# zeyadmohamedabdo/Visual-Question-Answering-VQA-system

Hardware: AMD Instinct MI355X
Metric: image-question pairs/sec (train step) (higher is better)
Workload: dtype bf16; 1 GPU; VQA train step fwd+CE+bwd+allreduce+clip+AdamW, batch 512/GPU, 3x224x224 images, 20 tokens, d=256, 4 text layers, 49 image tokens, 1000 answers, dropout on (BASELINE configs[2]); batch_per_gpu=512, global_batch=512, parallelism=dp1, reducer=off

## Files before the change

visual-question-answering-vqa-system_amd/csrc/token_ops.hip:

```cpp
#include <cstdlib>
#include "common.h"

template <typename T>
__global__ void embed_fwd_kernel(const long long* __restrict__ ids, const float* __restrict__ emb, const float* __restrict__ pe,
                                 T* __restrict__ out, int rows, int L, int D, int V, float scale, float p, uint64_t seed) {
  seed = drop_resolve(seed);
  const size_t i = (size_t)blockIdx.x * blockDim.x + threadIdx.x;
  if (i >= (size_t)rows * D) return;
  const int d = (int)(i % D), row = (int)(i / D), l = row % L;
  long long id = ids[row];
  float v = (id >= 0 && id < V) ? emb[(size_t)id * D + d] * scale : 0.f;
  v += pe[(size_t)l * D + d];
  if (p > 0.f) v = drop_keep32(drop_key(seed), (uint32_t)(i), p) ? v / (1.f - p) : 0.f;
  out[i] = from_f<T>(v);
}
__global__ __launch_bounds__(1024) void fold_rows_kernel(const float* __restrict__ part, int nrows, size_t stride, int ncols,
                                                         float* dst0, int n0, float* dst1) {
  const int c = blockIdx.x * 64 + threadIdx.x, rg = threadIdx.y;
  const int per = (nrows + 15) / 16, r0 = rg * per, r1 = min(nrows, r0 + per);
  float t = 0.f;
  if (c < ncols) {
    int r = r0;
    for (; r + 16 <= r1; r += 16) {
      float v[16];
// ... 802 lines not shown
  DT(hipLaunchKernelGGL((attn_fwd_kernel<float, true>), dim3(B * H), dim3(256), shm, st, (const float*)q, (const float*)k, (const float*)v, ldq, ldk, ldv, kmask, probs, (float*)ctx, ldc, H, Lq, Lk, hd, scale, 0.f, 0ull, kv_index, n_kv),
     hipLaunchKernelGGL((attn_fwd_kernel<bf16_t, true>), dim3(B * H), dim3(256), shm, st, (const bf16_t*)q, (const bf16_t*)k, (const bf16_t*)v, ldq, ldk, ldv, kmask, probs, (bf16_t*)ctx, ldc, H, Lq, Lk, hd, scale, 0.f, 0ull, kv_index, n_kv));
  VQA_LAUNCH_CHECK(); return VQA_OK;
}
int vqa_attention_bwd(int dtype, const void* dctx, int ldc, const void* q, const void* k, const void* v, int ldq, int ldk, int ldv,
                      const float* probs, void* dq, void* dk, void* dv, int lddq, int lddk, int lddv,
                      int B, int H, int Lq, int Lk, int hd, float p, unsigned long long seed, hipStream_t st) {
  return attention_bwd_valu<false>(dtype, dctx, ldc, q, k, v, ldq, ldk, ldv, probs, nullptr, dq, dk, dv, lddq, lddk, lddv, B, H, Lq, Lk, hd, p, seed, st);
}
int vqa_attention_bwd_dp(int dtype, const void* dctx, int ldc, const void* q, const void* k, const void* v, int ldq, int ldk, int ldv,
                         const float* probs, const float* dprobs, void* dq, void* dk, void* dv, int lddq, int lddk, int lddv,
                         int B, int H, int Lq, int Lk, int hd, float p, unsigned long long seed, hipStream_t st) {
  if (!dprobs) return VQA_EARG;
  return attention_bwd_valu<true>(dtype, dctx, ldc, q, k, v, ldq, ldk, ldv, probs, dprobs, dq, dk, dv, lddq, lddk, lddv, B, H, Lq, Lk, hd, p, seed, st);
}
int vqa_masked_pool_fwd(int dtype, const void* x, const float* mask, void* out, int ldo, int col0, int B, int L, int D, hipStream_t st) {
  DT(hipLaunchKernelGGL(masked_pool_fwd_kernel<float>, dim3(B), dim3(256), 0, st, (const float*)x, mask, (float*)out, ldo, col0, L, D),
     hipLaunchKernelGGL(masked_pool_fwd_kernel<bf16_t>, dim3(B), dim3(256), 0, st, (const bf16_t*)x, mask, (bf16_t*)out, ldo, col0, L, D));
  VQA_LAUNCH_CHECK(); return VQA_OK;
}
int vqa_masked_pool_pair_fwd(int dtype, const void* x0, const void* x1, const float* mask, void* out, int B, int L, int D, hipStream_t st) {
  if (!x0 || !x1 || !out || B <= 0 || L <= 0 || D <= 0) return VQA_EARG;
  DT(hipLaunchKernelGGL(masked_pool_pair_fwd_kernel<float>, dim3(B, 2), dim3(256), 0, st, (const float*)x0, (const float*)x1, mask, (float*)out, L, D),
     hipLaunchKernelGGL(masked_pool_pair_fwd_kernel<bf16_t>, dim3(B, 2), dim3(256), 0, st, (const bf16_t*)x0, (const bf16_t*)x1, mask, (bf16_t*)out, L, D));
  VQA_LAUNCH_CHECK(); return VQA_OK;
}
int vqa_masked_pool_pair_bwd(int dtype, const void* dcat, const float* mask, void* dx0, void* dx1, int B, int L, int D, hipStream_t st) {
  if (!dcat || !dx0 || !dx1 || B <= 0 || L <= 0 || D <= 0) return VQA_EARG;
  DT(hipLaunchKernelGGL(masked_pool_pair_bwd_kernel<float>, dim3(B, 2), dim3(256), 0, st, (const float*)dcat, mask, (float*)dx0, (float*)dx1, L, D),
     hipLaunchKernelGGL(masked_pool_pair_bwd_kernel<bf16_t>, dim3(B, 2), dim3(256), 0, st, (const bf16_t*)dcat, mask, (bf16_t*)dx0, (bf16_t*)dx1, L, D));
  VQA_LAUNCH_CHECK(); return VQA_OK;
}
int vqa_masked_pool_bwd(int dtype, const void* dpool, int ldo, int col0, const float* mask, const void* addend, void* dx, int B, int L, int D, hipStream_t st) {
  DT(hipLaunchKernelGGL(masked_pool_bwd_kernel<float>, dim3(B), dim3(256), 0, st, (const float*)dpool, ldo, col0, mask, (const float*)addend, (float*)dx, L, D),
     hipLaunchKernelGGL(masked_pool_bwd_kernel<bf16_t>, dim3(B), dim3(256), 0, st, (const bf16_t*)dpool, ldo, col0, mask, (const bf16_t*)addend, (bf16_t*)dx, L, D));
  VQA_LAUNCH_CHECK(); return VQA_OK;
}
int vqa_gate_fwd(int dtype, const void* z, const void* cat, void* fused, int B, int D, hipStream_t st) {
  DT(hipLaunchKernelGGL(gate_fwd_kernel<float>, dim3(g1((size_t)B * D)), dim3(256), 0, st, (const float*)z, (const float*)cat, (float*)fused, B, D),
     hipLaunchKernelGGL(gate_fwd_kernel<bf16_t>, dim3(g1((size_t)B * D)), dim3(256), 0, st, (const bf16_t*)z, (const bf16_t*)cat, (bf16_t*)fused, B, D));
  VQA_LAUNCH_CHECK(); return VQA_OK;
}
int vqa_gate_bwd(int dtype, const void* dfused, const void* z, const void* cat, void* dz, void* dcat, int B, int D, hipStream_t st) {
  DT(hipLaunchKernelGGL(gate_bwd_kernel<float>, dim3(g1((size_t)B * D)), dim3(256), 0, st, (const float*)dfused, (const float*)z, (const float*)cat, (float*)dz, (float*)dcat, B, D),
     hipLaunchKernelGGL(gate_bwd_kernel<bf16_t>, dim3(g1((size_t)B * D)), dim3(256), 0, st, (const bf16_t*)dfused, (const bf16_t*)z, (const bf16_t*)cat, (bf16_t*)dz, (bf16_t*)dcat, B, D));
  VQA_LAUNCH_CHECK(); return VQA_OK;
}
int vqa_grad_tap_add(int dtype, const float* g, void* acc, int rows, int cols, int ld, int layout, hipStream_t st) {
  if (!g || !acc || rows < 0 || cols <= 0 || ld <= 0) return VQA_EARG;
  if (rows == 0) return VQA_OK;
  if (layout == 0) {
    if (ld < cols) return VQA_EARG;
    const size_t n = (size_t)rows * cols;
    DT(hipLaunchKernelGGL(grad_tap_rows_kernel<float>, dim3(g1(n)), dim3(256), 0, st, g, (float*)acc, cols, ld, n),
       hipLaunchKernelGGL(grad_tap_rows_kernel<bf16_t>, dim3(g1(n)), dim3(256), 0, st, g, (bf16_t*)acc, cols, ld, n));
  } else if (layout == 1) {
    if (rows % ld) return VQA_EARG;
    const int B = rows / ld;
    if (B > 65535) return VQA_EARG;
    const dim3 grid((unsigned)((ld + 31) / 32), (unsigned)((cols + 63) / 64), (unsigned)B);
    DT(hipLaunchKernelGGL(grad_tap_nchw_kernel<float>, grid, dim3(256), 0, st, g, (float*)acc, cols, ld),
       hipLaunchKernelGGL(grad_tap_nchw_kernel<bf16_t>, grid, dim3(256), 0, st, g, (bf16_t*)acc, cols, ld));
  } else {
    return VQA_EARG;
  }
  VQA_LAUNCH_CHECK(); return VQA_OK;
}
int vqa_add(int dtype, const void* a, const void* b, void* out, long long n, hipStream_t st) {
  DT(hipLaunchKernelGGL(add_kernel<float>, dim3(g1((size_t)n)), dim3(256), 0, st, (const float*)a, (const float*)b, (float*)out, (size_t)n),
     hipLaunchKernelGGL(add_kernel<bf16_t>, dim3(g1((size_t)n)), dim3(256), 0, st, (const bf16_t*)a, (const bf16_t*)b, (bf16_t*)out, (size_t)n));
  VQA_LAUNCH_CHECK(); return VQA_OK;
}
struct BiasBwdGeom { bool vec; int gpb, rows_per; dim3 grid; };
static BiasBwdGeom bias_bwd_geom(int dtype, int M, int N) {
  BiasBwdGeom g;
  const int VEC = dtype ? 8 : 4;
  g.vec = N % VEC == 0 && M > 0 && (256 % (N / VEC < 256 ? N / VEC : 256)) == 0;
  if (g.vec) {
    const int cvs = N / VEC, gpb = cvs < 256 ? cvs : 256, lanes_r = 256 / gpb;
    int gy = (M + 4 * lanes_r - 1) / (4 * lanes_r);
    if (gy > 1024) gy = 1024;
    if (gy < 1) gy = 1;
    g.gpb = gpb; g.rows_per = (M + gy - 1) / gy;
    g.grid = dim3((cvs + gpb - 1) / gpb, (M + g.rows_per - 1) / g.rows_per);
  } else {
    int gy = (M + 127) / 128; if (gy > 256) gy = 256; if (gy < 1) gy = 1;
    g.gpb = 0; g.rows_per = 0; g.grid = dim3((N + 63) / 64, gy);
  }
  return g;
}
long long vqa_bias_act_bwd_ws(int dtype, int M, int N) {
  if (M <= 0 || N <= 0) return 0;
  const BiasBwdGeom g = bias_bwd_geom(dtype, M, N);
  return (long long)g.grid.y * N;
}
int vqa_bias_act_bwd_fold_rows(int dtype, int M, int N) {
  if (M <= 0 || N <= 0) return 0;
  return (int)bias_bwd_geom(dtype, M, N).grid.y;
}
int vqa_bias_act_bwd(int dtype, const void* dout, const void* outact, void* dz, float* dbias, int M, int N, float p, unsigned long long seed,
                     float* ws, int defer_fold, hipStream_t st) {
  if (M <= 0 || N <= 0 || (defer_fold && !ws)) return VQA_EARG;
  const BiasBwdGeom g = bias_bwd_geom(dtype, M, N);
  if (g.vec) {
    DT(hipLaunchKernelGGL(bias_act_bwd_vec_kernel<float>, g.grid, dim3(256), 0, st, (const float*)dout, (const float*)outact, (float*)dz, dbias, M, N, p, seed, g.rows_per, ws),
       hipLaunchKernelGGL(bias_act_bwd_vec_kernel<bf16_t>, g.grid, dim3(256), 0, st, (const bf16_t*)dout, (const bf16_t*)outact, (bf16_t*)dz, dbias, M, N, p, seed, g.rows_per, ws));
  } else {
    DT(hipLaunchKernelGGL(bias_act_bwd_kernel<float>, g.grid, dim3(256), 0, st, (const float*)dout, (const float*)outact, (float*)dz, dbias, M, N, 0, p, seed, ws),
       hipLaunchKernelGGL(bias_act_bwd_kernel<bf16_t>, g.grid, dim3(256), 0, st, (const bf16_t*)dout, (const bf16_t*)outact, (bf16_t*)dz, dbias, M, N, 0, p, seed, ws));
  }
  if (ws && dbias && !defer_fold) launch_fold(ws, (int)g.grid.y, (size_t)N, N, dbias, N, nullptr, st);
  VQA_LAUNCH_CHECK(); return VQA_OK;
}
int vqa_fold_group(int njobs, const float* const* part, const int* nrows, const long long* stride, const int* ncols, float* const* dst0,
                   const int* n0, float* const* dst1, hipStream_t st) {
  if (njobs <= 0 || !part || !nrows || !stride || !ncols || !dst0 || !n0 || !dst1) return VQA_EARG;
  for (int base = 0; base < njobs; base += FOLD_MAXJOBS) {
    FoldGroup g;
    g.n = njobs - base < FOLD_MAXJOBS ? njobs - base : FOLD_MAXJOBS;
    g.blk0[0] = 0;
    for (int q = 0; q < g.n; ++q) {
      const int j = base + q;
      if (!part[j] || !dst0[j] || nrows[j] <= 0 || ncols[j] <= 0 || stride[j] <= 0 || stride[j] > 0xffffffffll || (n0[j] < ncols[j] && !dst1[j]))
        return VQA_EARG;
      g.j[q] = FoldJob{part[j], dst0[j], dst1[j], nrows[j], ncols[j], n0[j], (unsigned)stride[j]};
      g.blk0[q + 1] = g.blk0[q] + (ncols[j] + 63) / 64;
    }
    hipLaunchKernelGGL(fold_group_kernel, dim3(g.blk0[g.n]), dim3(64, 16), 0, st, g);
  }
  VQA_LAUNCH_CHECK(); return VQA_OK;
}
int vqa_cross_entropy(int dtype, const void* logits, const long long* targets, float* loss, void* dlogits, float* logits_f32, int B, int N,
                      float gscale, int* err, float* ws, hipStream_t st) {
  if (!logits || !targets || B <= 0 || N <= 0) return VQA_EARG;
  dim3 grid((B + 3) / 4);
  DT(hipLaunchKernelGGL(cross_entropy_kernel<float>, grid, dim3(256), 0, st, (const float*)logits, targets, loss, (float*)dlogits, logits_f32, B, N, gscale, err, ws),
     hipLaunchKernelGGL(cross_entropy_kernel<bf16_t>, grid, dim3(256), 0, st, (const bf16_t*)logits, targets, loss, (bf16_t*)dlogits, logits_f32, B, N, gscale, err, ws));
  if (ws && loss) launch_fold(ws, B, 1, 1, loss, 1, nullptr, st);
  VQA_LAUNCH_CHECK(); return VQA_OK;
}
int vqa_convert(int dtype_in, int dtype_out, const void* in, void* out, long long n, hipStream_t st) {
  const unsigned g = g1((size_t)n);
  if (!dtype_in && dtype_out) hipLaunchKernelGGL((convert_kernel<float, bf16_t>), dim3(g), dim3(256), 0, st, (const float*)in, (bf16_t*)out, (size_t)n);
  else if (dtype_in && !dtype_out) hipLaunchKernelGGL((convert_kernel<bf16_t, float>), dim3(g), dim3(256), 0, st, (const bf16_t*)in, (float*)out, (size_t)n);
  else if (!dtype_in) hipLaunchKernelGGL((convert_kernel<float, float>), dim3(g), dim3(256), 0, st, (const float*)in, (float*)out, (size_t)n);
  else hipLaunchKernelGGL((convert_kernel<bf16_t, bf16_t>), dim3(g), dim3(256), 0, st, (const bf16_t*)in, (bf16_t*)out, (size_t)n);
  VQA_LAUNCH_CHECK(); return VQA_OK;
}

}

typedef __attribute__((ext_vector_type(16))) float f32x16;

template <int HD, int NKT, int WPB, bool IDX = false>
__global__ __launch_bounds__(WPB * 64, 1) void attn_fwd_mfma_kernel(const bf16_t* __restrict__ q, const bf16_t* __restrict__ k, const bf16_t* __restrict__ v,
                                                            int ldq, int ldk, int ldv, const float* __restrict__ kmask, float* __restrict__ probs,
                                                            bf16_t* __restrict__ ctx, int ldc, int BH, int H, int Lq, int Lk, float p, uint64_t seed,
                                                            const int* __restrict__ kv_index, int n_kv) {
  seed = drop_resolve(seed);
  constexpr int LDV = HD;
  constexpr int KR = NKT * 32;
  constexpr int LDP = KR + 1;
  extern __shared__ __attribute__((aligned(16))) char smem[];
  const int lane = threadIdx.x & 63, wave = threadIdx.x >> 6;
  const int bh = blockIdx.x * WPB + wave;
  bf16_t* Vs = reinterpret_cast<bf16_t*>(smem) + wave * (KR * LDV);
  float* Ps = reinterpret_cast<float*>(smem + WPB * KR * LDV * 2) + wave * (32 * LDP);
  if (bh >= BH) return;
  const int b = bh / H, h = bh - b * H;
  const int r = lane & 31, hh = lane >> 5;
  const float inv_scale = 1.0f / sqrtf((float)HD);
  int kb = b;
  if constexpr (IDX) {
    kb = __builtin_amdgcn_readfirstlane(kv_index[b]);
    if (kb < 0 || kb >= n_kv) {
      for (int i = lane; i < Lq * Lk; i += 64) probs[(size_t)bh * Lq * Lk + i] = NAN;
      for (int i = lane; i < Lq * HD; i += 64) ctx[(size_t)(b * Lq + i / HD) * ldc + h * HD + i % HD] = f2bf(NAN);
      return;
    }
  }

  for (int i = lane; i < KR * (HD / 8); i += 64) {
    const int row = i / (HD / 8), cv = i - row * (HD / 8);
    u32x4 val = {0u, 0u, 0u, 0u};
    if (row < Lk) val = *reinterpret_cast<const u32x4*>(v + (size_t)(kb * Lk + row) * ldv + h * HD + cv * 8);
    *reinterpret_cast<u32x4*>(&Vs[row * LDV + cv * 8]) = val;
  }
  f32x16 st[NKT];
#pragma unroll
  for (int t = 0; t < NKT; ++t)
#pragma unroll
    for (int e = 0; e < 16; ++e) st[t][e] = 0.f;
#pragma unroll
  for (int ks = 0; ks < HD / 16; ++ks) {
    bf16x8 qf = {};
    if (r < Lq) qf = *reinterpret_cast<const bf16x8*>(q + (size_t)(b * Lq + r) * ldq + h * HD + ks * 16 + 8 * hh);
#pragma unroll
    for (int t = 0; t < NKT; ++t) {
      bf16x8 kf = {};
      if (32 * t + r < Lk) kf = *reinterpret_cast<const bf16x8*>(k + (size_t)(kb * Lk + 32 * t + r) * ldk + h * HD + ks * 16 + 8 * hh);
      st[t] = __builtin_amdgcn_mfma_f32_32x32x16_bf16(kf, qf, st[t], 0, 0, 0);
    }
  }
  float m = -INFINITY;
#pragma unroll
  for (int t = 0; t < NKT; ++t)
#pragma unroll
    for (int e = 0; e < 16; ++e) {
      const int key = 32 * t + (e & 3) + 8 * (e >> 2) + 4 * hh;
      float s = st[t][e] * inv_scale;
      if (key >= Lk || (kmask && kmask[kb * Lk + key] == 0.f)) s = -INFINITY;
      st[t][e] = s;
      m = fmaxf(m, s);
    }
  m = fmaxf(m, __shfl_xor(m, 32, 64));
  float sum = 0.f;
#pragma unroll
  for (int t = 0; t < NKT; ++t)
#pragma unroll
    for (int e = 0; e < 16; ++e) { const float ex = expf(st[t][e] - m); st[t][e] = ex; sum += ex; }
  sum += __shfl_xor(sum, 32, 64);
  const float rs = 1.0f / sum;
  const size_t prow = ((size_t)bh * Lq + r) * Lk;
#pragma unroll
  for (int t = 0; t < NKT; ++t)
#pragma unroll
    for (int e = 0; e < 16; ++e) {
      const int key = 32 * t + (e & 3) + 8 * (e >> 2) + 4 * hh;
      float pr = st[t][e] * rs;
      if (sum != sum || m != m) pr = st[t][e] / sum;
      Ps[r * LDP + key] = pr;
      if (p > 0.f && r < Lq && key < Lk) pr = drop_keep32(drop_key(seed), (uint32_t)(prow + key), p) ? pr / (1.f - p) : 0.f;
      st[t][e] = pr;
    }
  asm volatile("s_waitcnt lgkmcnt(0)" ::: "memory");
  for (int i = lane; i < Lq * Lk; i += 64) { const int qi = i / Lk, kj = i - qi * Lk; probs[(size_t)bh * Lq * Lk + i] = Ps[qi * LDP + kj]; }
  f32x16 o[HD / 32];
#pragma unroll
  for (int c = 0; c < HD / 32; ++c)
#pragma unroll
    for (int e = 0; e < 16; ++e) o[c][e] = 0.f;
  const int g2 = (lane >> 4) & 1, li = lane & 15, qd = li >> 2, pp = li & 3;
  typedef __attribute__((ext_vector_type(8))) short i16x8;
#pragma unroll
  for (int t = 0; t < NKT; ++t)
#pragma unroll
    for (int s = 0; s < 2; ++s) {
      bf16x8 af;
#pragma unroll
      for (int jj = 0; jj < 8; ++jj) af[jj] = (__bf16)st[t][8 * s + jj];
#pragma unroll
      for (int c = 0; c < HD / 32; ++c) {
        const bf16_t* vb = Vs + (32 * t + 16 * s + 4 * hh + qd) * LDV + c * 32 + 16 * g2 + 4 * pp;
        i16x4 lo = __builtin_amdgcn_ds_read_tr16_b64_v4i16((i16x4 __attribute__((address_space(3)))*)(vb));
        i16x4 hi = __builtin_amdgcn_ds_read_tr16_b64_v4i16((i16x4 __attribute__((address_space(3)))*)(vb + 8 * LDV));
        i16x8 tt = {lo[0], lo[1], lo[2], lo[3], hi[0], hi[1], hi[2], hi[3]};
        o[c] = __builtin_amdgcn_mfma_f32_32x32x16_bf16(af, __builtin_bit_cast(bf16x8, tt), o[c], 0, 0, 0);
      }
    }
#pragma unroll
  for (int c = 0; c < HD / 32; ++c)
#pragma unroll
    for (int e = 0; e < 16; ++e) {
      const int qi = (e & 3) + 8 * (e >> 2) + 4 * hh;
      if (qi < Lq) ctx[(size_t)(b * Lq + qi) * ldc + h * HD + c * 32 + r] = f2bf(o[c][e]);
    }
}

extern "C" int vqa_attention_fwd_mfma(const void* q, const void* k, const void* v, int ldq, int ldk, int ldv, const float* kmask, float* probs,
                                      void* ctx, int ldc, int B, int H, int Lq, int Lk, int hd, float p, unsigned long long seed, hipStream_t st) {
  if (!q || !k || !v || !probs || !ctx || Lq > 32 || Lk > 160 || (hd != 32 && hd != 64) || (ldq % 8) || (ldk % 8) || (ldv % 8)) return VQA_EARG;
  const int BH = B * H;
  auto go = [&](auto kern, int nkt, int wpb) {
    const size_t shm = (size_t)wpb * (nkt * 32) * hd * 2 + (size_t)wpb * 32 * (nkt * 32 + 1) * 4;
    (void)vqa_ensure_lds(reinterpret_cast<const void*>(kern), shm);
    hipLaunchKernelGGL(kern, dim3((BH + wpb - 1) / wpb), dim3(wpb * 64), shm, st, (const bf16_t*)q, (const bf16_t*)k, (const bf16_t*)v, ldq, ldk, ldv,
                       kmask, probs, (bf16_t*)ctx, ldc, BH, H, Lq, Lk, p, seed, nullptr, 0);
  };
  if (Lk <= 64) { if (hd == 32) go(&attn_fwd_mfma_kernel<32, 2, 4>, 2, 4); else go(&attn_fwd_mfma_kernel<64, 2, 4>, 2, 4); }
  else { if (hd == 32) go(&attn_fwd_mfma_kernel<32, 5, 2>, 5, 2); else go(&attn_fwd_mfma_kernel<64, 5, 2>, 5, 2); }
  VQA_LAUNCH_CHECK(); return VQA_OK;
}

extern "C" int vqa_attention_fwd_mfma_idx(const void* q, const void* k, const void* v, int ldq, int ldk, int ldv, const int* kv_index, int n_kv,
                                          const float* kmask, float* probs, void* ctx, int ldc, int B, int H, int Lq, int Lk, int hd, hipStream_t st) {
  if (!q || !k || !v || !kv_index || n_kv < 0 || !probs || !ctx || Lq > 32 || Lk > 160 || (hd != 32 && hd != 64) || (ldq % 8) || (ldk % 8) || (ldv % 8))
    return VQA_EARG;
  const int BH = B * H;
  auto go = [&](auto kern, int nkt, int wpb) {
    const size_t shm = (size_t)wpb * (nkt * 32) * hd * 2 + (size_t)wpb * 32 * (nkt * 32 + 1) * 4;
    (void)vqa_ensure_lds(reinterpret_cast<const void*>(kern), shm);
    hipLaunchKernelGGL(kern, dim3((BH + wpb - 1) / wpb), dim3(wpb * 64), shm, st, (const bf16_t*)q, (const bf16_t*)k, (const bf16_t*)v, ldq, ldk, ldv,
                       kmask, probs, (bf16_t*)ctx, ldc, BH, H, Lq, Lk, 0.f, 0ull, kv_index, n_kv);
  };
  if (Lk <= 64) { if (hd == 32) go(&attn_fwd_mfma_kernel<32, 2, 4, true>, 2, 4); else go(&attn_fwd_mfma_kernel<64, 2, 4, true>, 2, 4); }
  else { if (hd == 32) go(&attn_fwd_mfma_kernel<32, 5, 2, true>, 5, 2); else go(&attn_fwd_mfma_kernel<64, 5, 2, true>, 5, 2); }
  VQA_LAUNCH_CHECK(); return VQA_OK;
}

template <int HD>
__device__ __forceinline__ bf16x8 attn_ldsB(const bf16_t* tile, int row0, int c, int hh, int g2, int qd, int pp) {
  typedef __attribute__((ext_vector_type(8))) short i16x8;
  const bf16_t* vb = tile + (row0 + 4 * hh + qd) * HD + c * 32 + 16 * g2 + 4 * pp;
  i16x4 lo = __builtin_amdgcn_ds_read_tr16_b64_v4i16((i16x4 __attribute__((address_space(3)))*)(vb));
  i16x4 hi = __builtin_amdgcn_ds_read_tr16_b64_v4i16((i16x4 __attribute__((address_space(3)))*)(vb + 8 * HD));
  i16x8 tt = {lo[0], lo[1], lo[2], lo[3], hi[0], hi[1], hi[2], hi[3]};
  return __builtin_bit_cast(bf16x8, tt);
}

template <int HD, int NKT, int WPB, bool DPR>
__global__ __launch_bounds__(WPB * 64, 1) void attn_bwd_mfma_kernel(const bf16_t* __restrict__ dctx, int ldc, const bf16_t* __restrict__ q,
                                                            const bf16_t* __restrict__ k, const bf16_t* __restrict__ v, int ldq, int ldk, int ldv,
                                                            const float* __restrict__ probs, bf16_t* __restrict__ dq, bf16_t* __restrict__ dk,
                                                            bf16_t* __restrict__ dv, int lddq, int lddk, int lddv, int BH, int H, int Lq, int Lk,
                                                            float p, uint64_t seed, const float* __restrict__ dprobs) {
  seed = drop_resolve(seed);
  constexpr int KR = NKT * 32;
  constexpr int LDP = KR + 1;
  constexpr int WAVE_BYTES = (KR + 32 + 32) * HD * 2 + 32 * LDP * 4 + 32 * 4 + (DPR ? 32 * LDP * 4 : 0);
  extern __shared__ __attribute__((aligned(16))) char smem[];
  const int lane = threadIdx.x & 63, wave = threadIdx.x >> 6;
  const int bh = blockIdx.x * WPB + wave;
  if (bh >= BH) return;
  char* base = smem + (size_t)wave * WAVE_BYTES;
  bf16_t* Ks = reinterpret_cast<bf16_t*>(base);
  bf16_t* Qs = Ks + KR * HD;
  bf16_t* Os = Qs + 32 * HD;
  float* Ps = reinterpret_cast<float*>(Os + 32 * HD);
  float* Ts = Ps + 32 * LDP;
  float* DPs = Ts + 32;
  const int b = bh / H, h = bh - b * H;
  const int r = lane & 31, hh = lane >> 5;
  const int g2 = (lane >> 4) & 1, li = lane & 15, qd = li >> 2, pp = li & 3;
  const float inv_scale = 1.0f / sqrtf((float)HD);
  const float keep = p > 0.f ? 1.f / (1.f - p) : 1.f;

  for (int i = lane; i < KR * (HD / 8); i += 64) {
    const int row = i / (HD / 8), cv = i - row * (HD / 8);
    u32x4 val = {0u, 0u, 0u, 0u};
    if (row < Lk) val = *reinterpret_cast<const u32x4*>(k + (size_t)(b * Lk + row) * ldk + h * HD + cv * 8);
    *reinterpret_cast<u32x4*>(&Ks[row * HD + cv * 8]) = val;
  }
  for (int i = lane; i < 32 * (HD / 8); i += 64) {
    const int row = i / (HD / 8), cv = i - row * (HD / 8);
    u32x4 a = {0u, 0u, 0u, 0u}, o = {0u, 0u, 0u, 0u};
    if (row < Lq) {
      a = *reinterpret_cast<const u32x4*>(q + (size_t)(b * Lq + row) * ldq + h * HD + cv * 8);
      o = *reinterpret_cast<const u32x4*>(dctx + (size_t)(b * Lq + row) * ldc + h * HD + cv * 8);
    }
    *reinterpret_cast<u32x4*>(&Qs[row * HD + cv * 8]) = a;
    *reinterpret_cast<u32x4*>(&Os[row * HD + cv * 8]) = o;
  }
  for (int i = lane; i < Lq * Lk; i += 64) { const int qi = i / Lk, kj = i - qi * Lk; Ps[qi * LDP + kj] = probs[(size_t)bh * Lq * Lk + i]; }
  if constexpr (DPR)
    for (int i = lane; i < Lq * Lk; i += 64) { const int qi = i / Lk, kj = i - qi * Lk; DPs[qi * LDP + kj] = dprobs[(size_t)bh * Lq * Lk + i]; }

  f32x16 d1[NKT], d2[NKT];
#pragma unroll
  for (int t = 0; t < NKT; ++t)
#pragma unroll
    for (int e = 0; e < 16; ++e) { d1[t][e] = 0.f; d2[t][e] = 0.f; }
#pragma unroll
  for (int ks = 0; ks < HD / 16; ++ks) {
    bf16x8 of = {};
    if (r < Lq) of = *reinterpret_cast<const bf16x8*>(dctx + (size_t)(b * Lq + r) * ldc + h * HD + ks * 16 + 8 * hh);
#pragma unroll
    for (int t = 0; t < NKT; ++t) {
      bf16x8 vf = {};
      if (32 * t + r < Lk) vf = *reinterpret_cast<const bf16x8*>(v + (size_t)(b * Lk + 32 * t + r) * ldv + h * HD + ks * 16 + 8 * hh);
      d1[t] = __builtin_amdgcn_mfma_f32_32x32x16_bf16(vf, of, d1[t], 0, 0, 0);
      d2[t] = __builtin_amdgcn_mfma_f32_32x32x16_bf16(of, vf, d2[t], 0, 0, 0);
    }
  }
  asm volatile("s_waitcnt lgkmcnt(0)" ::: "memory");

  const size_t prow = ((size_t)bh * Lq + r) * Lk;
  float tq = 0.f;
#pragma unroll
  for (int t = 0; t < NKT; ++t)
#pragma unroll
    for (int e = 0; e < 16; ++e) {
      const int key = 32 * t + (e & 3) + 8 * (e >> 2) + 4 * hh;
      const bool ok = r < Lq && key < Lk;
      const float pr = ok ? Ps[r * LDP + key] : 0.f;
      float ks = 1.f;
      if (p > 0.f && ok) ks = drop_keep32(drop_key(seed), (uint32_t)(prow + key), p) ? keep : 0.f;
      float dp = ok ? d1[t][e] * ks : 0.f;
      if constexpr (DPR) dp += ok ? DPs[r * LDP + key] : 0.f;
      tq += dp * pr;
      d1[t][e] = dp;
    }
  tq += __shfl_xor(tq, 32, 64);
  if (hh == 0) Ts[r] = tq;
#pragma unroll
  for (int t = 0; t < NKT; ++t)
#pragma unroll
    for (int e = 0; e < 16; ++e) {
      const int key = 32 * t + (e & 3) + 8 * (e >> 2) + 4 * hh;
      const float pr = (r < Lq && key < Lk) ? Ps[r * LDP + key] : 0.f;
      d1[t][e] = pr * (d1[t][e] - tq) * inv_scale;
    }
  asm volatile("s_waitcnt lgkmcnt(0)" ::: "memory");
  f32x16 oq[HD / 32];
#pragma unroll
  for (int c = 0; c < HD / 32; ++c)
#pragma unroll
    for (int e = 0; e < 16; ++e) oq[c][e] = 0.f;
#pragma unroll
  for (int t = 0; t < NKT; ++t)
#pragma unroll
    for (int s2 = 0; s2 < 2; ++s2) {
      bf16x8 af;
#pragma unroll
      for (int jj = 0; jj < 8; ++jj) af[jj] = (__bf16)d1[t][8 * s2 + jj];
#pragma unroll
      for (int c = 0; c < HD / 32; ++c)
        oq[c] = __builtin_amdgcn_mfma_f32_32x32x16_bf16(af, attn_ldsB<HD>(Ks, 32 * t + 16 * s2, c, hh, g2, qd, pp), oq[c], 0, 0, 0);
    }
#pragma unroll
  for (int c = 0; c < HD / 32; ++c)
#pragma unroll
    for (int e = 0; e < 16; ++e) {
      const int qi = (e & 3) + 8 * (e >> 2) + 4 * hh;
      if (qi < Lq) dq[(size_t)(b * Lq + qi) * lddq + h * HD + c * 32 + r] = f2bf(oq[c][e]);
    }

#pragma unroll
  for (int t = 0; t < NKT; ++t) {
    const int key = 32 * t + r;
    f32x16 ds2, pd2;
#pragma unroll
    for (int e = 0; e < 16; ++e) {
      const int qi = (e & 3) + 8 * (e >> 2) + 4 * hh;
      const bool ok = qi < Lq && key < Lk;
      const float pr = ok ? Ps[qi * LDP + key] : 0.f;
      float ks = 1.f;
      if (p > 0.f && ok) ks = drop_keep32(drop_key(seed), (uint32_t)(((size_t)bh * Lq + qi) * Lk + key), p) ? keep : 0.f;
      float dp = ok ? d2[t][e] * ks : 0.f;
      if constexpr (DPR) dp += ok ? DPs[qi * LDP + key] : 0.f;
      const float tt = ok ? Ts[qi] : 0.f;
      ds2[e] = pr * (dp - tt) * inv_scale;
      pd2[e] = pr * ks;
    }
// ... 722 lines not shown
    for (int ks = 0; ks < HD / 16; ++ks) {
      bf16x8 of = {};
      if (r < Lq) of = *reinterpret_cast<const bf16x8*>(dctx + (size_t)(b * Lq + r) * ldc + h * HD + ks * 16 + 8 * hh);
#pragma unroll
      for (int t = 0; t < NKT; ++t) {
        bf16x8 vf = {};
        if (32 * t + r < Lk) vf = *reinterpret_cast<const bf16x8*>(v + (size_t)(u * Lk + 32 * t + r) * ldv + h * HD + ks * 16 + 8 * hh);
        d1[t] = __builtin_amdgcn_mfma_f32_32x32x16_bf16(vf, of, d1[t], 0, 0, 0);
        d2[t] = __builtin_amdgcn_mfma_f32_32x32x16_bf16(of, vf, d2[t], 0, 0, 0);
      }
    }
    asm volatile("s_waitcnt lgkmcnt(0)" ::: "memory");

    const size_t prow = ((size_t)bh * Lq + r) * Lk;
    float tq = 0.f;
#pragma unroll
    for (int t = 0; t < NKT; ++t)
#pragma unroll
      for (int e = 0; e < 16; ++e) {
        const int key = 32 * t + (e & 3) + 8 * (e >> 2) + 4 * hh;
        const bool ok = r < Lq && key < Lk;
        const float pr = ok ? Ps[r * LDP + key] : 0.f;
        float ks = 1.f;
        if (p > 0.f && ok) ks = drop_keep32(drop_key(seed), (uint32_t)(prow + key), p) ? keep : 0.f;
        const float dp = ok ? d1[t][e] * ks : 0.f;
        tq += dp * pr;
        d1[t][e] = dp;
      }
    tq += __shfl_xor(tq, 32, 64);
    if (hh == 0) Ts[r] = tq;
#pragma unroll
    for (int t = 0; t < NKT; ++t)
#pragma unroll
      for (int e = 0; e < 16; ++e) {
        const int key = 32 * t + (e & 3) + 8 * (e >> 2) + 4 * hh;
        const float pr = (r < Lq && key < Lk) ? Ps[r * LDP + key] : 0.f;
        d1[t][e] = pr * (d1[t][e] - tq) * inv_scale;
      }
    asm volatile("s_waitcnt lgkmcnt(0)" ::: "memory");
    f32x16 oq[HD / 32];
#pragma unroll
    for (int c = 0; c < HD / 32; ++c)
#pragma unroll
      for (int e = 0; e < 16; ++e) oq[c][e] = 0.f;
#pragma unroll
    for (int t = 0; t < NKT; ++t)
#pragma unroll
      for (int s2 = 0; s2 < 2; ++s2) {
        bf16x8 af;
#pragma unroll
        for (int jj = 0; jj < 8; ++jj) af[jj] = (__bf16)d1[t][8 * s2 + jj];
#pragma unroll
        for (int c = 0; c < HD / 32; ++c)
          oq[c] = __builtin_amdgcn_mfma_f32_32x32x16_bf16(af, attn_ldsB<HD>(Ks, 32 * t + 16 * s2, c, hh, g2, qd, pp), oq[c], 0, 0, 0);
      }
#pragma unroll
    for (int c = 0; c < HD / 32; ++c)
#pragma unroll
      for (int e = 0; e < 16; ++e) {
        const int qi = (e & 3) + 8 * (e >> 2) + 4 * hh;
        if (qi < Lq) dq[(size_t)(b * Lq + qi) * lddq + h * HD + c * 32 + r] = f2bf(oq[c][e]);
      }

#pragma unroll
    for (int t = 0; t < NKT; ++t) {
      const int key = 32 * t + r;
      f32x16 ds2, pd2;
#pragma unroll
      for (int e = 0; e < 16; ++e) {
        const int qi = (e & 3) + 8 * (e >> 2) + 4 * hh;
        const bool ok = qi < Lq && key < Lk;
        const float pr = ok ? Ps[qi * LDP + key] : 0.f;
        float ks = 1.f;
        if (p > 0.f && ok) ks = drop_keep32(drop_key(seed), (uint32_t)(((size_t)bh * Lq + qi) * Lk + key), p) ? keep : 0.f;
        const float dp = ok ? d2[t][e] * ks : 0.f;
        const float tt = ok ? Ts[qi] : 0.f;
        ds2[e] = pr * (dp - tt) * inv_scale;
        pd2[e] = pr * ks;
      }
      f32x16 okk[HD / 32], ovv[HD / 32];
#pragma unroll
      for (int c = 0; c < HD / 32; ++c)
#pragma unroll
        for (int e = 0; e < 16; ++e) {
          const int a = ((t * (HD / 32) + c) * 16 + e) * 64 + lane;
          okk[c][e] = Ak[a]; ovv[c][e] = Av[a];
        }
#pragma unroll
      for (int s2 = 0; s2 < 2; ++s2) {
        bf16x8 as, ap;
#pragma unroll
        for (int jj = 0; jj < 8; ++jj) { as[jj] = (__bf16)ds2[8 * s2 + jj]; ap[jj] = (__bf16)pd2[8 * s2 + jj]; }
#pragma unroll
        for (int c = 0; c < HD / 32; ++c) {
          okk[c] = __builtin_amdgcn_mfma_f32_32x32x16_bf16(as, attn_ldsB<HD>(Qs, 16 * s2, c, hh, g2, qd, pp), okk[c], 0, 0, 0);
          ovv[c] = __builtin_amdgcn_mfma_f32_32x32x16_bf16(ap, attn_ldsB<HD>(Os, 16 * s2, c, hh, g2, qd, pp), ovv[c], 0, 0, 0);
        }
      }
#pragma unroll
      for (int c = 0; c < HD / 32; ++c)
#pragma unroll
        for (int e = 0; e < 16; ++e) {
          const int a = ((t * (HD / 32) + c) * 16 + e) * 64 + lane;
          Ak[a] = okk[c][e]; Av[a] = ovv[c][e];
        }
    }
  }
  asm volatile("s_waitcnt lgkmcnt(0)" ::: "memory");
  for (int t = 0; t < NKT; ++t)
#pragma unroll
    for (int c = 0; c < HD / 32; ++c)
#pragma unroll
      for (int e = 0; e < 16; ++e) {
        const int kj = 32 * t + (e & 3) + 8 * (e >> 2) + 4 * hh;
        const int a = ((t * (HD / 32) + c) * 16 + e) * 64 + lane;
        if (kj < Lk) {
          dk[(size_t)(u * Lk + kj) * lddk + h * HD + c * 32 + r] = f2bf(Ak[a]);
          dv[(size_t)(u * Lk + kj) * lddv + h * HD + c * 32 + r] = f2bf(Av[a]);
        }
      }
}

extern "C" {

int vqa_index_csr(const int* kv_index, int N, int U, int* offsets, int* order, hipStream_t st) {
  if (N < 0 || U < 0 || U > 32768 || !offsets || (N > 0 && (!kv_index || !order))) return VQA_EARG;
  const size_t shm = (size_t)(U > 0 ? U : 1) * 4;
  (void)vqa_ensure_lds(reinterpret_cast<const void*>(&index_csr_kernel), shm);
  hipLaunchKernelGGL(index_csr_kernel, dim3(1), dim3(1024), shm, st, kv_index, N, U, offsets, order);
  VQA_LAUNCH_CHECK(); return VQA_OK;
}

int vqa_attention_fwd_idx_train(int dtype, const void* q, const void* k, const void* v, int ldq, int ldk, int ldv, const int* kv_index,
                                int n_kv, const float* kmask, float* probs, void* ctx, int ldc, int B, int H, int Lq, int Lk, int hd,
                                float p, unsigned long long seed, hipStream_t st) {
  if (!kv_index || n_kv < 0 || !(p >= 0.f && p < 1.f)) return VQA_EARG;
  const size_t shm = ((size_t)(Lq + 2 * Lk) * (hd + 1) + (size_t)Lq * (Lk + 1)) * 4;
  if (shm > 160 * 1024) return VQA_EARG;
  const float scale = sqrtf((float)hd);
  (void)vqa_ensure_lds(dtype ? reinterpret_cast<const void*>(&attn_fwd_kernel<bf16_t, true>) : reinterpret_cast<const void*>(&attn_fwd_kernel<float, true>), shm);
  DT(hipLaunchKernelGGL((attn_fwd_kernel<float, true>), dim3(B * H), dim3(256), shm, st, (const float*)q, (const float*)k, (const float*)v, ldq, ldk, ldv, kmask, probs, (float*)ctx, ldc, H, Lq, Lk, hd, scale, p, seed, kv_index, n_kv),
     hipLaunchKernelGGL((attn_fwd_kernel<bf16_t, true>), dim3(B * H), dim3(256), shm, st, (const bf16_t*)q, (const bf16_t*)k, (const bf16_t*)v, ldq, ldk, ldv, kmask, probs, (bf16_t*)ctx, ldc, H, Lq, Lk, hd, scale, p, seed, kv_index, n_kv));
  VQA_LAUNCH_CHECK(); return VQA_OK;
}

int vqa_attention_fwd_mfma_idx_train(const void* q, const void* k, const void* v, int ldq, int ldk, int ldv, const int* kv_index, int n_kv,
                                     const float* kmask, float* probs, void* ctx, int ldc, int B, int H, int Lq, int Lk, int hd, float p,
                                     unsigned long long seed, hipStream_t st) {
  if (!q || !k || !v || !kv_index || n_kv < 0 || !probs || !ctx || Lq > 32 || Lk > 160 || (hd != 32 && hd != 64) || (ldq % 8) || (ldk % 8) ||
      (ldv % 8) || !(p >= 0.f && p < 1.f))
    return VQA_EARG;
  const int BH = B * H;
  auto go = [&](auto kern, int nkt, int wpb) {
    const size_t shm = (size_t)wpb * (nkt * 32) * hd * 2 + (size_t)wpb * 32 * (nkt * 32 + 1) * 4;
    (void)vqa_ensure_lds(reinterpret_cast<const void*>(kern), shm);
    hipLaunchKernelGGL(kern, dim3((BH + wpb - 1) / wpb), dim3(wpb * 64), shm, st, (const bf16_t*)q, (const bf16_t*)k, (const bf16_t*)v, ldq, ldk, ldv,
                       kmask, probs, (bf16_t*)ctx, ldc, BH, H, Lq, Lk, p, seed, kv_index, n_kv);
  };
  if (Lk <= 64) { if (hd == 32) go(&attn_fwd_mfma_kernel<32, 2, 4, true>, 2, 4); else go(&attn_fwd_mfma_kernel<64, 2, 4, true>, 2, 4); }
  else { if (hd == 32) go(&attn_fwd_mfma_kernel<32, 5, 2, true>, 5, 2); else go(&attn_fwd_mfma_kernel<64, 5, 2, true>, 5, 2); }
  VQA_LAUNCH_CHECK(); return VQA_OK;
}

int vqa_attention_bwd_idx(int dtype, const void* dctx, int ldc, const void* q, const void* k, const void* v, int ldq, int ldk, int ldv,
                          const float* probs, const int* offsets, const int* order, int n_kv, void* dq, void* dk, void* dv,
                          int lddq, int lddk, int lddv, int B, int H, int Lq, int Lk, int hd, float p, unsigned long long seed,
                          hipStream_t st) {
  if (!dctx || !q || !k || !v || !probs || !offsets || (B > 0 && !order) || !dq || !dk || !dv || n_kv < 0 || B < 0 || H <= 0 ||
      Lq <= 0 || Lk <= 0 || hd <= 0 || !(p >= 0.f && p < 1.f))
    return VQA_EARG;
  const size_t shm = ((size_t)(2 * Lq + 2 * Lk) * (hd + 1) + (size_t)2 * Lq * (Lk + 1)) * 4;
  const long long nkd = (long long)Lk * hd;
  if (shm > 160 * 1024 || nkd > 256 * 40) return VQA_EARG;
  if (n_kv == 0) return VQA_OK;
  const float scale = sqrtf((float)hd);
  auto go = [&](auto kf, auto kb) {
    (void)vqa_ensure_lds(dtype ? reinterpret_cast<const void*>(kb) : reinterpret_cast<const void*>(kf), shm);
    DT(hipLaunchKernelGGL(kf, dim3(n_kv * H), dim3(256), shm, st, (const float*)dctx, ldc, (const float*)q, (const float*)k, (const float*)v, ldq, ldk, ldv, probs, (float*)dq, (float*)dk, (float*)dv, lddq, lddk, lddv, H, Lq, Lk, hd, scale, p, seed, offsets, order, B),
       hipLaunchKernelGGL(kb, dim3(n_kv * H), dim3(256), shm, st, (const bf16_t*)dctx, ldc, (const bf16_t*)q, (const bf16_t*)k, (const bf16_t*)v, ldq, ldk, ldv, probs, (bf16_t*)dq, (bf16_t*)dk, (bf16_t*)dv, lddq, lddk, lddv, H, Lq, Lk, hd, scale, p, seed, offsets, order, B));
  };
  if (nkd <= 256 * 16) go(&attn_bwd_idx_kernel<float, 16>, &attn_bwd_idx_kernel<bf16_t, 16>);
  else go(&attn_bwd_idx_kernel<float, 40>, &attn_bwd_idx_kernel<bf16_t, 40>);
  VQA_LAUNCH_CHECK(); return VQA_OK;
}

int vqa_attention_bwd_mfma_idx(const void* dctx, int ldc, const void* q, const void* k, const void* v, int ldq, int ldk, int ldv,
                               const float* probs, const int* offsets, const int* order, int n_kv, void* dq, void* dk, void* dv,
                               int lddq, int lddk, int lddv, int B, int H, int Lq, int Lk, int hd, float p, unsigned long long seed,
                               hipStream_t st) {
  if (!dctx || !q || !k || !v || !probs || !offsets || (B > 0 && !order) || !dq || !dk || !dv || n_kv < 0 || B < 0 || H <= 0 ||
      Lq <= 0 || Lq > 32 || Lk <= 0 || Lk > 160 || (hd != 32 && hd != 64) || (ldq % 8) || (ldk % 8) || (ldv % 8) || (ldc % 8) ||
      !(p >= 0.f && p < 1.f))
    return VQA_EARG;
  if (n_kv == 0) return VQA_OK;
  const int UH = n_kv * H;
  auto go = [&](auto kern, int nkt, int wpb) {
    const size_t nacc = (size_t)nkt * (hd / 32) * 16;
    const size_t shm = (size_t)wpb * ((nkt * 32 + 32 + 32) * hd * 2 + 32 * (nkt * 32 + 1) * 4 + 32 * 4 + 2 * nacc * 64 * 4);
    (void)vqa_ensure_lds(reinterpret_cast<const void*>(kern), shm);
    hipLaunchKernelGGL(kern, dim3((UH + wpb - 1) / wpb), dim3(wpb * 64), shm, st, (const bf16_t*)dctx, ldc, (const bf16_t*)q, (const bf16_t*)k,
                       (const bf16_t*)v, ldq, ldk, ldv, probs, (bf16_t*)dq, (bf16_t*)dk, (bf16_t*)dv, lddq, lddk, lddv, UH, H, Lq, Lk, p, seed,
                       offsets, order, B);
  };
  if (Lk <= 64) { if (hd == 32) go(&attn_bwd_mfma_idx_kernel<32, 2, 2>, 2, 2); else go(&attn_bwd_mfma_idx_kernel<64, 2, 2>, 2, 2); }
  else { if (hd == 32) go(&attn_bwd_mfma_idx_kernel<32, 5, 1>, 5, 1); else go(&attn_bwd_mfma_idx_kernel<64, 5, 1>, 5, 1); }
  VQA_LAUNCH_CHECK(); return VQA_OK;
}

}
```

Baseline: 41860 pairs/s.

## Restructure MFMA attention forward: prefetch Q/K/V, ballot key mask, compact LDS, coalesced stores

The forward MFMA attention kernel now issues all V, Q and K global loads up front into registers before any MFMA, so memory latency overlaps. It converts the key mask into per-lane bitmasks with a ballot instead of reloading it per element. The probability tile in LDS is sized to the real Lq x Lk, and the context output is staged through LDS and written as 16-byte rows. Launch bounds allow four blocks per CU for the short-key case. The cost is higher register pressure from the prefetched fragments, plus extra LDS waits.

```diff
diff --git a/visual-question-answering-vqa-system_amd/csrc/token_ops.hip b/visual-question-answering-vqa-system_amd/csrc/token_ops.hip
--- a/visual-question-answering-vqa-system_amd/csrc/token_ops.hip
+++ b/visual-question-answering-vqa-system_amd/csrc/token_ops.hip
@@ -978,20 +978,36 @@
 
 typedef __attribute__((ext_vector_type(16))) float f32x16;
 
+__host__ __device__ inline int attn_ps_bytes(int Lq, int Lk) { return Lq > 0 && Lk > 0 ? (Lq * (Lk | 1) * 4 + 15) & ~15 : 0; }
+static size_t attn_fwd_lds(int wpb, int nkt, int hd, int Lq, int Lk) { return (size_t)wpb * ((size_t)nkt * 32 * hd * 2 + attn_ps_bytes(Lq, Lk)); }
+
+template <int HD>
+__device__ __forceinline__ void attn_store_rows(const bf16_t* tile, bf16_t* dst, int ld, int nrows, int lane) {
+  if (!(ld & 7) && !(reinterpret_cast<uintptr_t>(dst) & 15)) {
+    for (int i = lane; i < nrows * (HD / 8); i += 64) {
+      const int row = i / (HD / 8), cv = i - row * (HD / 8);
+      *reinterpret_cast<u32x4*>(dst + (size_t)row * ld + cv * 8) = *reinterpret_cast<const u32x4*>(&tile[row * HD + cv * 8]);
+    }
+  } else {
+    for (int i = lane; i < nrows * HD; i += 64) { const int row = i / HD, d = i - row * HD; dst[(size_t)row * ld + d] = tile[row * HD + d]; }
+  }
+}
+
 template <int HD, int NKT, int WPB, bool IDX = false>
-__global__ __launch_bounds__(WPB * 64, 1) void attn_fwd_mfma_kernel(const bf16_t* __restrict__ q, const bf16_t* __restrict__ k, const bf16_t* __restrict__ v,
+__global__ __launch_bounds__(WPB * 64, NKT == 2 ? 4 : 1) void attn_fwd_mfma_kernel(const bf16_t* __restrict__ q, const bf16_t* __restrict__ k, const bf16_t* __restrict__ v,
                                                             int ldq, int ldk, int ldv, const float* __restrict__ kmask, float* __restrict__ probs,
                                                             bf16_t* __restrict__ ctx, int ldc, int BH, int H, int Lq, int Lk, float p, uint64_t seed,
                                                             const int* __restrict__ kv_index, int n_kv) {
   seed = drop_resolve(seed);
   constexpr int LDV = HD;
   constexpr int KR = NKT * 32;
-  constexpr int LDP = KR + 1;
+  constexpr int NV = KR * (HD / 8) / 64;
+  const int LDP = Lk | 1;
   extern __shared__ __attribute__((aligned(16))) char smem[];
   const int lane = threadIdx.x & 63, wave = threadIdx.x >> 6;
   const int bh = blockIdx.x * WPB + wave;
   bf16_t* Vs = reinterpret_cast<bf16_t*>(smem) + wave * (KR * LDV);
-  float* Ps = reinterpret_cast<float*>(smem + WPB * KR * LDV * 2) + wave * (32 * LDP);
+  float* Ps = reinterpret_cast<float*>(smem + WPB * KR * LDV * 2 + wave * attn_ps_bytes(Lq, Lk));
   if (bh >= BH) return;
   const int b = bh / H, h = bh - b * H;
   const int r = lane & 31, hh = lane >> 5;
@@ -1006,11 +1022,41 @@
     }
   }
 
-  for (int i = lane; i < KR * (HD / 8); i += 64) {
-    const int row = i / (HD / 8), cv = i - row * (HD / 8);
-    u32x4 val = {0u, 0u, 0u, 0u};
-    if (row < Lk) val = *reinterpret_cast<const u32x4*>(v + (size_t)(kb * Lk + row) * ldv + h * HD + cv * 8);
-    *reinterpret_cast<u32x4*>(&Vs[row * LDV + cv * 8]) = val;
+  u32x4 vreg[NV];
+#pragma unroll
+  for (int j = 0; j < NV; ++j) {
+    const int i = lane + 64 * j, row = i / (HD / 8), cv = i - row * (HD / 8);
+    vreg[j] = u32x4{0u, 0u, 0u, 0u};
+    if (row < Lk) vreg[j] = *reinterpret_cast<const u32x4*>(v + (size_t)(kb * Lk + row) * ldv + h * HD + cv * 8);
+  }
+  bf16x8 qf[HD / 16], kf[HD / 16][NKT];
+#pragma unroll
+  for (int ks = 0; ks < HD / 16; ++ks) {
+    qf[ks] = bf16x8{};
+    if (r < Lq) qf[ks] = *reinterpret_cast<const bf16x8*>(q + (size_t)(b * Lq + r) * ldq + h * HD + ks * 16 + 8 * hh);
+#pragma unroll
+    for (int t = 0; t < NKT; ++t) {
+      kf[ks][t] = bf16x8{};
+      if (32 * t + r < Lk) kf[ks][t] = *reinterpret_cast<const bf16x8*>(k + (size_t)(kb * Lk + 32 * t + r) * ldk + h * HD + ks * 16 + 8 * hh);
+    }
+  }
+  float mval[(NKT + 1) / 2];
+#pragma unroll
+  for (int c = 0; c < (NKT + 1) / 2; ++c) {
+    mval[c] = 1.f;
+    if (kmask && 64 * c + lane < Lk) mval[c] = kmask[kb * Lk + 64 * c + lane];
+  }
+#pragma unroll
+  for (int j = 0; j < NV; ++j) {
+    const int i = lane + 64 * j, row = i / (HD / 8), cv = i - row * (HD / 8);
+    *reinterpret_cast<u32x4*>(&Vs[row * LDV + cv * 8]) = vreg[j];
+  }
+  uint32_t mbits[NKT];
+#pragma unroll
+  for (int c = 0; c < (NKT + 1) / 2; ++c) {
+    const unsigned long long bal = __ballot(64 * c + lane >= Lk || mval[c] == 0.f);
+    mbits[2 * c] = (uint32_t)bal >> (4 * hh);
+    if (2 * c + 1 < NKT) mbits[2 * c + 1] = (uint32_t)(bal >> 32) >> (4 * hh);
   }
   f32x16 st[NKT];
 #pragma unroll
@@ -1018,24 +1064,16 @@
 #pragma unroll
     for (int e = 0; e < 16; ++e) st[t][e] = 0.f;
 #pragma unroll
-  for (int ks = 0; ks < HD / 16; ++ks) {
-    bf16x8 qf = {};
-    if (r < Lq) qf = *reinterpret_cast<const bf16x8*>(q + (size_t)(b * Lq + r) * ldq + h * HD + ks * 16 + 8 * hh);
-#pragma unroll
-    for (int t = 0; t < NKT; ++t) {
-      bf16x8 kf = {};
-      if (32 * t + r < Lk) kf = *reinterpret_cast<const bf16x8*>(k + (size_t)(kb * Lk + 32 * t + r) * ldk + h * HD + ks * 16 + 8 * hh);
-      st[t] = __builtin_amdgcn_mfma_f32_32x32x16_bf16(kf, qf, st[t], 0, 0, 0);
-    }
-  }
+  for (int ks = 0; ks < HD / 16; ++ks)
+#pragma unroll
+    for (int t = 0; t < NKT; ++t) st[t] = __builtin_amdgcn_mfma_f32_32x32x16_bf16(kf[ks][t], qf[ks], st[t], 0, 0, 0);
   float m = -INFINITY;
 #pragma unroll
   for (int t = 0; t < NKT; ++t)
 #pragma unroll
     for (int e = 0; e < 16; ++e) {
-      const int key = 32 * t + (e & 3) + 8 * (e >> 2) + 4 * hh;
       float s = st[t][e] * inv_scale;
-      if (key >= Lk || (kmask && kmask[kb * Lk + key] == 0.f)) s = -INFINITY;
+      if ((mbits[t] >> ((e & 3) + 8 * (e >> 2))) & 1u) s = -INFINITY;
       st[t][e] = s;
       m = fmaxf(m, s);
     }
@@ -1055,12 +1093,23 @@
       const int key = 32 * t + (e & 3) + 8 * (e >> 2) + 4 * hh;
       float pr = st[t][e] * rs;
       if (sum != sum || m != m) pr = st[t][e] / sum;
-      Ps[r * LDP + key] = pr;
-      if (p > 0.f && r < Lq && key < Lk) pr = drop_keep32(drop_key(seed), (uint32_t)(prow + key), p) ? pr / (1.f - p) : 0.f;
+      if (r < Lq && key < Lk) {
+        Ps[r * LDP + key] = pr;
+        if (p > 0.f) pr = drop_keep32(drop_key(seed), (uint32_t)(prow + key), p) ? pr / (1.f - p) : 0.f;
+      }
       st[t][e] = pr;
     }
   asm volatile("s_waitcnt lgkmcnt(0)" ::: "memory");
-  for (int i = lane; i < Lq * Lk; i += 64) { const int qi = i / Lk, kj = i - qi * Lk; probs[(size_t)bh * Lq * Lk + i] = Ps[qi * LDP + kj]; }
+  {
+    const int total = Lq * Lk, pad = LDP - Lk, dq = 64 / Lk, dr = 64 - dq * Lk;
+    float* pout = probs + (size_t)bh * Lq * Lk;
+    int qi = lane / Lk, kj = lane - qi * Lk;
+    for (int i = lane; i < total; i += 64) {
+      pout[i] = Ps[i + qi * pad];
+      qi += dq; kj += dr;
+      if (kj >= Lk) { kj -= Lk; ++qi; }
+    }
+  }
   f32x16 o[HD / 32];
 #pragma unroll
   for (int c = 0; c < HD / 32; ++c)
@@ -1084,13 +1133,16 @@
         o[c] = __builtin_amdgcn_mfma_f32_32x32x16_bf16(af, __builtin_bit_cast(bf16x8, tt), o[c], 0, 0, 0);
       }
     }
+  asm volatile("s_waitcnt lgkmcnt(0)" ::: "memory");
 #pragma unroll
   for (int c = 0; c < HD / 32; ++c)
 #pragma unroll
     for (int e = 0; e < 16; ++e) {
       const int qi = (e & 3) + 8 * (e >> 2) + 4 * hh;
-      if (qi < Lq) ctx[(size_t)(b * Lq + qi) * ldc + h * HD + c * 32 + r] = f2bf(o[c][e]);
-    }
+      if (qi < Lq) Vs[qi * HD + c * 32 + r] = f2bf(o[c][e]);
+    }
+  asm volatile("s_waitcnt lgkmcnt(0)" ::: "memory");
+  attn_store_rows<HD>(Vs, ctx + (size_t)b * Lq * ldc + h * HD, ldc, Lq, lane);
 }
 
 extern "C" int vqa_attention_fwd_mfma(const void* q, const void* k, const void* v, int ldq, int ldk, int ldv, const float* kmask, float* probs,
@@ -1098,7 +1150,7 @@
   if (!q || !k || !v || !probs || !ctx || Lq > 32 || Lk > 160 || (hd != 32 && hd != 64) || (ldq % 8) || (ldk % 8) || (ldv % 8)) return VQA_EARG;
   const int BH = B * H;
   auto go = [&](auto kern, int nkt, int wpb) {
-    const size_t shm = (size_t)wpb * (nkt * 32) * hd * 2 + (size_t)wpb * 32 * (nkt * 32 + 1) * 4;
+    const size_t shm = attn_fwd_lds(wpb, nkt, hd, Lq, Lk);
     (void)vqa_ensure_lds(reinterpret_cast<const void*>(kern), shm);
     hipLaunchKernelGGL(kern, dim3((BH + wpb - 1) / wpb), dim3(wpb * 64), shm, st, (const bf16_t*)q, (const bf16_t*)k, (const bf16_t*)v, ldq, ldk, ldv,
                        kmask, probs, (bf16_t*)ctx, ldc, BH, H, Lq, Lk, p, seed, nullptr, 0);
@@ -1114,7 +1166,7 @@
     return VQA_EARG;
   const int BH = B * H;
   auto go = [&](auto kern, int nkt, int wpb) {
-    const size_t shm = (size_t)wpb * (nkt * 32) * hd * 2 + (size_t)wpb * 32 * (nkt * 32 + 1) * 4;
+    const size_t shm = attn_fwd_lds(wpb, nkt, hd, Lq, Lk);
     (void)vqa_ensure_lds(reinterpret_cast<const void*>(kern), shm);
     hipLaunchKernelGGL(kern, dim3((BH + wpb - 1) / wpb), dim3(wpb * 64), shm, st, (const bf16_t*)q, (const bf16_t*)k, (const bf16_t*)v, ldq, ldk, ldv,
                        kmask, probs, (bf16_t*)ctx, ldc, BH, H, Lq, Lk, 0.f, 0ull, kv_index, n_kv);
@@ -2143,7 +2195,7 @@
     return VQA_EARG;
   const int BH = B * H;
   auto go = [&](auto kern, int nkt, int wpb) {
-    const size_t shm = (size_t)wpb * (nkt * 32) * hd * 2 + (size_t)wpb * 32 * (nkt * 32 + 1) * 4;
+    const size_t shm = attn_fwd_lds(wpb, nkt, hd, Lq, Lk);
     (void)vqa_ensure_lds(reinterpret_cast<const void*>(kern), shm);
     hipLaunchKernelGGL(kern, dim3((BH + wpb - 1) / wpb), dim3(wpb * 64), shm, st, (const bf16_t*)q, (const bf16_t*)k, (const bf16_t*)v, ldq, ldk, ldv,
                        kmask, probs, (bf16_t*)ctx, ldc, BH, H, Lq, Lk, p, seed, kv_index, n_kv);
```

New measurement: 41910 pairs/s (median of 5 runs). Within noise of the previous version (+0.1%).
